# mila-iqia/diffusion_for_multi_scale_molecular_dynamics

Hardware: AMD Instinct MI355X
Metric: sampled structures/sec (1000-step predictor-corrector SDE sampling) (higher is better)
Workload: dtype f32 (per-edge matrix products as split-f16 hi/lo x3 MFMA terms with f32 accumulation: 22-bit products; state, updates, reductions and every other layer in f32)

## Files before the change

diffusion_for_multi_scale_molecular_dynamics_amd/csrc/mdx_egnn_chain.hip:

```cpp
#include <hip/hip_runtime.h>
#include <stdint.h>

#include <type_traits>

#include "../../include/mdx_hip.h"

namespace {

typedef _Float16 half8 __attribute__((ext_vector_type(8)));
typedef _Float16 half2v __attribute__((ext_vector_type(2)));
typedef float f32x16 __attribute__((ext_vector_type(16)));
typedef float f32x4 __attribute__((ext_vector_type(4)));
typedef __attribute__((address_space(3))) char lds_c;
typedef __attribute__((address_space(3))) float lds_f;
typedef __attribute__((address_space(1))) const char gbl_c;

constexpr int kWave = 64;
constexpr int kWaves = 4;
constexpr int kTileEdges = 32 * kWaves;
constexpr int kFastD = 6;
constexpr int kRing = 4;
constexpr int kScaleSlots = MDX_EGNN_CHAIN_MAX_LAYERS + 4;
constexpr int kMaxPositions = MDX_EGNN_CHAIN_MAX_LAYERS + 2;
constexpr int kEnds = kScaleSlots - 1;
// ... 995 lines not shown
            }
        };
        auto finish_rows = [&](Act<H, PREC>& y, Act<H, PREC>& u) {
            epilogue_elements<H, PREC>(NT - 1, 0, 16, pend, y, sc_prev, true, amax);
            flush_max(layers);
            const bool project = MODE == 3 && p.proj_out != nullptr;
            const float kOut = end_factor(2);
            int64_t row[NS];
            if constexpr (MODE == 3) {
#pragma unroll
                for (int es = 0; es < NS; ++es) row[es] = p.residual ? source_row(es, false) : e[es];
            }
#pragma unroll
            for (int q8 = 0; q8 < H / 8; ++q8) {
                const int t = q8 >> 2, q = q8 & 3, es = L::es(q), off = 32 * t + L::fb(q, h);
                f32x4 v = get4<H>(y, t, q);
#pragma unroll
                for (int i = 0; i < 4; ++i) v[i] *= kOut;
                if constexpr (SPLIT) {
#pragma unroll
                    for (int i = 0; i < 4; ++i) out_of_range = out_of_range || (is_live(es) && !(__builtin_fabsf(v[i]) <= 3.0e38f));
                }
                if (is_live(es)) {
                    if (p.residual) {
                        const f32x4 r4 = *(const f32x4*)(p.residual + (MODE == 3 ? row[es] : e[es]) * p.ld_in + off);
#pragma unroll
                        for (int i = 0; i < 4; ++i) v[i] = r4[i] + v[i];
                    }
                    *(f32x4*)(p.rows_out + e[es] * H + off) = v;
                }
                if ((q8 & 7) == 7) __builtin_amdgcn_sched_barrier(0);
            }
            ch.stores_count = stores_issued(H / 8);
            if constexpr (MODE == 3) {
                if (project) {
                    asm volatile("s_waitcnt vmcnt(0)" ::: "memory");
                    const float kIn = end_factor(3);
#pragma unroll
                    for (int q8 = 0; q8 < H / 8; ++q8) {
                        const int es = L::es(q8 & 3), off = 32 * (q8 >> 2) + L::fb(q8 & 3, h);
                        const f32x4 a = *(const f32x4*)(p.rows_out + e[es] * H + off);
                        note4(a[0] * kIn, a[1] * kIn, a[2] * kIn, a[3] * kIn);
                        put_pair<H>(u, q8 >> 2, 4 * (q8 & 3), a[0] * kIn, a[1] * kIn);
                        put_pair<H>(u, q8 >> 2, 4 * (q8 & 3) + 2, a[2] * kIn, a[3] * kIn);
                        if ((q8 & 15) == 15) __builtin_amdgcn_sched_barrier(0);
                    }
                    flush_max(layers + 1);
#pragma unroll 1
                    for (int t2 = 0; t2 < 2 * NT; ++t2) {
                        if constexpr (C::SPREAD) ch.scalar_addresses();
                        const f32x16 acc = run_tile(u, false, 0, u, t2 + 1 < 2 * NT ? nullptr : par, sc_prev);
                        const float to_out = load_scale(layers + t2 / NT).out;
#pragma unroll
                        for (int q = 0; q < 4; ++q) {
                            const int es = L::es(q);
                            const f32x4 v = {acc[4 * q] * to_out, acc[4 * q + 1] * to_out, acc[4 * q + 2] * to_out, acc[4 * q + 3] * to_out};
                            if constexpr (SPLIT) {
#pragma unroll
                                for (int i = 0; i < 4; ++i) out_of_range = out_of_range || (is_live(es) && !(__builtin_fabsf(v[i]) <= 3.0e38f));
                            }
                            if (is_live(es)) *(f32x4*)(p.proj_out + e[es] * 2 * H + 32 * t2 + L::fb(q, h)) = v;
                        }
                        ch.stores_count = stores_issued(4);
                    }
                }
            }
        };
        int l_first = 1;
        if constexpr (MODE == 3) {
#pragma unroll
            for (int t = 0; t < NT; ++t) {
                const f32x16 acc = run_tile(xa, false, 0, xa, t + 1 < NT ? par + 32 * (t + 1) : nullptr, sc_prev);
                park(xb, t, acc);
            }
            const float kIn = end_factor(1);
#pragma unroll
            for (int q8 = 0; q8 < H / 8; ++q8) {
                const int es = L::es(q8 & 3), off = 32 * (q8 >> 2) + L::fb(q8 & 3, h);
                const f32x4 a = *(const f32x4*)(p.rows_in2 + e[es] * p.ld_in2 + off);
                if constexpr (SPLIT) {
                    put_pair<H>(xa, q8 >> 2, 4 * (q8 & 3), a[0] * kIn, a[1] * kIn);
                    put_pair<H>(xa, q8 >> 2, 4 * (q8 & 3) + 2, a[2] * kIn, a[3] * kIn);
                } else {
                    note4(a[0] * kIn, a[1] * kIn, a[2] * kIn, a[3] * kIn);
#pragma unroll
                    for (int i = 0; i < 4; ++i) put<H>(xa, q8 >> 2, 4 * (q8 & 3) + i, a[i] * kIn);
                }
                if ((q8 & 15) == 15) __builtin_amdgcn_sched_barrier(0);
            }
            flush_max(0);
            acc_next = unpark(xb, 0);
#pragma unroll
            for (int t = 0; t < NT; ++t) {
                const lds_f* after = t + 1 < NT ? nullptr : par + 2 * H;
                pend = run_tile(xa, t > 0, t - 1, xb, after, sc_prev);
                if (t + 1 < NT) acc_next = unpark(xb, t + 1);
            }
            l_first = 2;
        } else {
            layer(std::true_type{}, xa, xb, 0);
        }
        bool done = false;
        if constexpr (MODE == 1) {
            if (layers == 1) {
                finish_rows(xb, xa);
                done = true;
            }
        }
        if (!done) {
            auto step_layer = [&](Act<H, PREC>& in, Act<H, PREC>& out, int l) {
                if constexpr (ATT) {
                    if (l == p.n_message) {
                        gate_messages(in, l);
                        reload_prefetch(par + l * H);
                        layer(std::true_type{}, in, out, l);
                    } else {
                        layer(std::false_type{}, in, out, l);
                    }
                } else {
                    layer(std::false_type{}, in, out, l);
                }
            };
            for (int l = l_first;;) {
                step_layer(xb, xa, l);
                if (!ROWS && l == p.n_message) {
                    if constexpr (MODE == 2) {
                        MDX_STAMP_ALWAYS(30);
                        ch.stores_count = aggregate_pieces(xb);
                        reload_prefetch(l + 1 < layers ? par + (l + 1) * H : nullptr);
                        MDX_STAMP_ALWAYS(31);
                    } else {
                        store_messages(xb);
                    }
                }
                if (++l >= layers) {
                    if constexpr (!ROWS) head_tile(xa);
                    else finish_rows(xa, xb);
                    break;
                }
                step_layer(xa, xb, l);
                if (!ROWS && l == p.n_message) {
                    if constexpr (MODE == 2) {
                        MDX_STAMP_ALWAYS(30);
                        ch.stores_count = aggregate_pieces(xa);
                        reload_prefetch(l + 1 < layers ? par + (l + 1) * H : nullptr);
                        MDX_STAMP_ALWAYS(31);
                    } else {
                        store_messages(xa);
                    }
                }
                if (++l >= layers) {
                    if constexpr (!ROWS) head_tile(xb);
                    else finish_rows(xb, xa);
                    break;
                }
            }
        }
    }
    asm volatile("s_waitcnt vmcnt(0)" ::: "memory");
    MDX_STAMP_ALWAYS(22);
    MDX_STAMP_REALTIME(23);
    if constexpr (SPLIT) {
        if (p.status && out_of_range) atomicOr(p.status, MDX_STATUS_EGNN_F16_RANGE);
    } else {
        __syncthreads();
        if (p.act_max && (int)threadIdx.x < layers + 2 && max_table[threadIdx.x]) atomicMax(p.act_max + threadIdx.x, max_table[threadIdx.x]);
    }
}

struct PackArgs {
    const float* w[MDX_EGNN_CHAIN_MAX_LAYERS];
    const float* w_out;
    int layers, H, precision;
    uint32_t tied;
    int32_t* exps;
    void* image;
};

__global__ __launch_bounds__(256) void egnn_chain_maxabs_kernel(PackArgs p)
{
    const int l = blockIdx.y;
    const bool head = l == p.layers;
    const float* w = head ? p.w_out : p.w[l];
    const int64_t n = head ? p.H : (int64_t)p.H * p.H;
    uint32_t m = 0;
    if (w)
        for (int64_t i = blockIdx.x * (int64_t)blockDim.x + threadIdx.x; i < n; i += (int64_t)gridDim.x * blockDim.x) {
            const uint32_t b = __builtin_bit_cast(uint32_t, w[i]) & 0x7fffffffu;
            if (b < 0x7f800000u && b > m) m = b;
        }
    for (int d = 32; d >= 1; d >>= 1) {
        const uint32_t o = (uint32_t)__shfl_xor((int)m, d);
        m = o > m ? o : m;
    }
    if ((threadIdx.x & 63) == 0 && m) atomicMax((uint32_t*)p.exps + l, m);
}
__global__ void egnn_chain_exponents_kernel(PackArgs p)
{
    if (blockIdx.x || threadIdx.x) return;
    for (int l = 0; l <= p.layers; ++l) {
        const uint32_t b = ((const uint32_t*)p.exps)[l];
        int a = 0;
        if (b) {
            const int e = (int)(b >> 23) - 127;
            a = 13 - (e < -126 ? -126 : e);
            a = a > 40 ? 40 : (a < -40 ? -40 : a);
        }
        p.exps[l] = a;
    }
    for (int l = 1; l < p.layers; ++l)
        if (p.tied >> l & 1u) {
            int lo = l - 1;
            while (lo > 0 && (p.tied >> lo & 1u)) --lo;
            int a = p.exps[lo];
            for (int k = lo + 1; k <= l; ++k) a = p.exps[k] < a ? p.exps[k] : a;
            for (int k = lo; k <= l; ++k) p.exps[k] = a;
        }
}

constexpr int kMinActExp = -14;
__global__ void egnn_chain_act_exponents_kernel(uint32_t* maxima, int count, int32_t* exps)
{
    if (blockIdx.x || threadIdx.x) return;
    for (int q = 0; q < count; ++q) {
        const uint32_t b = maxima[q] & 0x7fffffffu;
        maxima[q] = 0;
        if (!b) continue;
        const int e = b >= 0x7f800000u ? 127 : (int)(b >> 23) - 127;
        int c = 12 - e;
        c = c > kActExp<1> ? kActExp<1> : (c < kMinActExp ? kMinActExp : c);
        if (c < exps[q]) exps[q] = c;
    }
}

__global__ __launch_bounds__(256) void egnn_chain_pack_kernel(PackArgs p)
{
    const int H = p.H, NT = H / 32;
    const int64_t per_layer = (int64_t)H * H;
    const int64_t total = per_layer * p.layers + 32 * H;
    for (int64_t idx = blockIdx.x * (int64_t)blockDim.x + threadIdx.x; idx < total; idx += (int64_t)gridDim.x * blockDim.x) {
        const int l = (int)(idx / per_layer);
        int64_t r = idx - l * per_layer;
        const int t = (int)(r / (32 * H));
        r -= (int64_t)t * 32 * H;
        (void)NT;
        const bool head = l == p.layers;
        auto weight = [&](int n, int k) -> float {
            if (head) return (n == 0 && p.w_out) ? p.w_out[k] : 0.0f;
            return p.w[l][(int64_t)n * H + k];
        };
        if (p.precision == 0) {
            const int q = (int)(r / 256), lane = (int)(r % 256) / 4, i = (int)(r % 4);
            const int n = 32 * t + (lane & 31), k = 8 * q + 4 * (lane >> 5) + i;
            ((float*)p.image)[idx] = weight(n, k);
        } else {
            const int s = (int)(r / 512), lane = (int)(r % 512) / 8, j = (int)(r % 8);
            const int n = p.precision == 1 ? 32 * t + (lane & 31) : 32 * t + 16 * (s & 1) + (lane & 15);
            const int k = p.precision == 1 ? 16 * s + 8 * (j >> 2) + 4 * (lane >> 5) + (j & 3)
                                           : 32 * (s >> 1) + 16 * (j >> 2) + 4 * (lane >> 4) + (j & 3);
            const float v = weight(n, k) * pow2_bits(p.exps[l]);
            const _Float16 hi = (_Float16)v;
            const _Float16 lo = (_Float16)(v - (float)hi);
            _Float16* chunk = (_Float16*)((char*)p.image + ((int64_t)l * (H / 32) + t) * ((int64_t)H * 32 * 4));
            chunk[s * 1024 + lane * 8 + j] = hi;
            chunk[s * 1024 + 512 + lane * 8 + j] = lo;
        }
    }
}

__device__ __forceinline__ float coord_head_value(float s, int flags) { return (flags & MDX_EGNN_COORD_TANH) ? tanhf(s) : s; }
__device__ __forceinline__ float normalize_factor(float r2) { return tanhf(r2) / sqrtf(r2 + 1.0e-16f); }

__global__ __launch_bounds__(256) void egnn_coord_aggregate_kernel(const float* __restrict__ s, const float* __restrict__ coord,
                                                                   const int64_t* __restrict__ edges,
                                                                   const int64_t* __restrict__ offsets,
                                                                   const int64_t* __restrict__ degree, int64_t n_nodes, int D,
                                                                   int mean, int flags, float* __restrict__ out)
{
    const int64_t total = n_nodes * D;
    for (int64_t idx = blockIdx.x * (int64_t)blockDim.x + threadIdx.x; idx < total; idx += (int64_t)gridDim.x * blockDim.x) {
        const int64_t node = idx / D;
        const int k = (int)(idx - node * D);
        const int64_t e0 = offsets[node], deg = degree[node];
        const float ci = coord[idx];
        float acc = 0.0f;
        for (int64_t e = e0; e < e0 + deg; ++e) {
            const int64_t dst = edges[2 * e + 1];
            float diff = ci - coord[dst * D + k];
            if (flags & MDX_EGNN_COORD_NORMALIZE) {
                float r2 = 0.0f;
                for (int j = 0; j < D; ++j) {
                    const float dj = coord[node * D + j] - coord[dst * D + j];
                    r2 += dj * dj;
                }
                diff = normalize_factor(r2) * diff;
            }
            acc += diff * coord_head_value(s[e], flags);
        }
        if (mean && deg > 0) acc = acc / (float)deg;
        out[idx] = ci + acc;
    }
}

__global__ __launch_bounds__(256) void segment_combine_kernel(const float* __restrict__ pieces, const int64_t* __restrict__ offsets,
                                                              const int64_t* __restrict__ degree, int64_t n_nodes, int H,
                                                              int mean, float* __restrict__ out, const float* __restrict__ left,
                                                              int64_t boundary_rows)
{
    const int lane = threadIdx.x % kWave;
    const int64_t wave = (blockIdx.x * (int64_t)blockDim.x + threadIdx.x) / kWave;
    const int64_t n_waves = ((int64_t)gridDim.x * blockDim.x) / kWave;
    const int quads = H >> 2;
    for (int64_t node = wave; node < n_nodes; node += n_waves) {
        const int64_t e0 = offsets[node], deg = degree[node], e1 = e0 + deg;
        const float count = (mean && deg > 0) ? (float)deg : 1.0f;
        const int64_t last_row = ((e1 - 1) & 15) == 15 ? ((e1 - 1) >> 4) : boundary_rows + node;
        for (int q = lane; q < quads; q += kWave) {
            f32x4 acc = {0.0f, 0.0f, 0.0f, 0.0f};
            for (int64_t e = e0 | 15; e < e1 - 1; e += 16) acc += reinterpret_cast<const f32x4*>(pieces + (e >> 4) * H)[q];
            if (deg > 0) acc += reinterpret_cast<const f32x4*>(pieces + last_row * H)[q];
            if (mean) acc = acc / count;
            if (left) {
                reinterpret_cast<f32x4*>(out + node * 2 * H)[q] = reinterpret_cast<const f32x4*>(left + node * H)[q];
                reinterpret_cast<f32x4*>(out + node * 2 * H + H)[q] = acc;
            } else {
                reinterpret_cast<f32x4*>(out + node * H)[q] = acc;
            }
        }
    }
}

__global__ __launch_bounds__(256) void egnn_node_gather_kernel(const float* __restrict__ pieces, const int64_t* __restrict__ offsets,
                                                               const int64_t* __restrict__ degree, int64_t n_nodes, int H,
                                                               int mean_messages, float* __restrict__ out,
                                                               const float* __restrict__ left, int64_t boundary_rows,
                                                               const float* __restrict__ s, const float* __restrict__ coord,
                                                               const int64_t* __restrict__ edges, int D, int mean_coords,
                                                               int flags, float* __restrict__ coord_out)
{
    const int lane = threadIdx.x % kWave;
    const int64_t wave = (blockIdx.x * (int64_t)blockDim.x + threadIdx.x) / kWave;
    const int64_t n_waves = ((int64_t)gridDim.x * blockDim.x) / kWave;
    const int quads = H >> 2;
    for (int64_t node = wave; node < n_nodes; node += n_waves) {
        const int64_t e0 = offsets[node], deg = degree[node], e1 = e0 + deg;
        float part[8] = {0, 0, 0, 0, 0, 0, 0, 0}, ci[8];
#pragma unroll
        for (int k = 0; k < 8; ++k) ci[k] = k < D ? coord[node * D + k] : 0.0f;
        for (int64_t e = e0 + lane; e < e1; e += kWave) {
            const int64_t dst = edges[2 * e + 1];
            const float se = coord_head_value(s[e], flags);
            if (flags & MDX_EGNN_COORD_NORMALIZE) {
                float diff[8], r2 = 0.0f;
#pragma unroll
                for (int k = 0; k < 8; ++k) {
                    diff[k] = k < D ? ci[k] - coord[dst * D + k] : 0.0f;
                    if (k < D) r2 += diff[k] * diff[k];
                }
                const float f = normalize_factor(r2);
#pragma unroll
                for (int k = 0; k < 8; ++k)
                    if (k < D) part[k] += (f * diff[k]) * se;
            } else {
#pragma unroll
                for (int k = 0; k < 8; ++k)
                    if (k < D) part[k] += (ci[k] - coord[dst * D + k]) * se;
            }
        }
        const float count = (mean_messages && deg > 0) ? (float)deg : 1.0f;
        const int64_t last_row = ((e1 - 1) & 15) == 15 ? ((e1 - 1) >> 4) : boundary_rows + node;
        for (int q = lane; pieces && q < quads; q += kWave) {
            f32x4 acc = {0.0f, 0.0f, 0.0f, 0.0f};
            for (int64_t e = e0 | 15; e < e1 - 1; e += 16) acc += reinterpret_cast<const f32x4*>(pieces + (e >> 4) * H)[q];
            if (deg > 0) acc += reinterpret_cast<const f32x4*>(pieces + last_row * H)[q];
            if (mean_messages) acc = acc / count;
            if (left) {
                reinterpret_cast<f32x4*>(out + node * 2 * H)[q] = reinterpret_cast<const f32x4*>(left + node * H)[q];
                reinterpret_cast<f32x4*>(out + node * 2 * H + H)[q] = acc;
            } else {
                reinterpret_cast<f32x4*>(out + node * H)[q] = acc;
            }
        }
#pragma unroll
        for (int k = 0; k < 8; ++k) {
            if (k < D) {
                float v = part[k];
                v += __builtin_bit_cast(float, __builtin_amdgcn_update_dpp(0, __builtin_bit_cast(int, v), 0x111, 0xf, 0xf, false));
                v += __builtin_bit_cast(float, __builtin_amdgcn_update_dpp(0, __builtin_bit_cast(int, v), 0x112, 0xf, 0xf, false));
                v += __builtin_bit_cast(float, __builtin_amdgcn_update_dpp(0, __builtin_bit_cast(int, v), 0x114, 0xf, 0xf, false));
                v += __builtin_bit_cast(float, __builtin_amdgcn_update_dpp(0, __builtin_bit_cast(int, v), 0x118, 0xf, 0xf, false));
                v += __builtin_bit_cast(float, __builtin_amdgcn_update_dpp(0, __builtin_bit_cast(int, v), 0x142, 0xa, 0xf, false));
                v += __builtin_bit_cast(float, __builtin_amdgcn_update_dpp(0, __builtin_bit_cast(int, v), 0x143, 0xc, 0xf, false));
                part[k] = __builtin_bit_cast(float, __builtin_amdgcn_readlane(__builtin_bit_cast(int, v), 63));
            }
        }
        if (lane < D) {
            float total = 0.0f, mine = 0.0f;
#pragma unroll
            for (int k = 0; k < 8; ++k) {
                if (k == lane) { total = part[k]; mine = ci[k]; }
            }
            if (mean_coords && deg > 0) total = total / (float)deg;
            coord_out[node * D + lane] = mine + total;
        }
    }
}

template <int H, int PREC, int MODE, bool ATT = false>
int launch_chain(const ChainArgs& a, int layers, hipStream_t st)
{
    using C = Chain<H, PREC>;
    size_t lds = (size_t)kRing * C::CHUNK + sizeof(float) * ((size_t)layers * H + 2 * H + 4 * kScaleSlots) +
                 sizeof(int) * kWaves * 32 + sizeof(uint32_t) * kMaxPositions;
    if (ATT) lds = ((lds + 15) & ~(size_t)15) + sizeof(float) * (H + 4);
    static bool granted[64] = {};
    int dev = 0;
    if (hipGetDevice(&dev) != hipSuccess || dev < 0 || dev >= 64) return MDX_ERR_HIP;
    if (lds > 64 * 1024 && !granted[dev]) {
        if (hipFuncSetAttribute((const void*)egnn_edge_chain_kernel<H, PREC, MODE, ATT>, hipFuncAttributeMaxDynamicSharedMemorySize,
                                160 * 1024) != hipSuccess)
            return MDX_ERR_HIP;
        granted[dev] = true;
    }
    if (lds > 160 * 1024) return MDX_ERR_UNSUPPORTED;
    int64_t tiles = (a.n_edges + kTileEdges - 1) / kTileEdges;
    int cus = 256;
    if (hipDeviceGetAttribute(&cus, hipDeviceAttributeMultiprocessorCount, dev) != hipSuccess) cus = 256;
    const unsigned grid = (unsigned)(tiles < cus ? tiles : cus);
    hipLaunchKernelGGL((egnn_edge_chain_kernel<H, PREC, MODE, ATT>), dim3(grid), dim3(kWaves * kWave), lds, st, a);
    return hipGetLastError() == hipSuccess ? MDX_OK : MDX_ERR_HIP;
}

}

extern "C" int mdx_chain_launch_attention(const void* args, int hidden, int precision, int layers, mdx_stream_t stream);

#ifdef MDX_CHAIN_ATTENTION_UNIT
extern "C" int mdx_chain_launch_attention(const void* args, int hidden, int precision, int layers, mdx_stream_t stream)
{
    const ChainArgs& a = *static_cast<const ChainArgs*>(args);
    hipStream_t st = reinterpret_cast<hipStream_t>(stream);
#define MDX_ATT_CASE(HH) \
    case HH: return precision == 0 ? launch_chain<HH, 0, 2, true>(a, layers, st) : (precision == 1 ? launch_chain<HH, 1, 2, true>(a, layers, st) : launch_chain<HH, 2, 2, true>(a, layers, st));
    switch (hidden) {
        MDX_ATT_CASE(32)
        MDX_ATT_CASE(64)
        MDX_ATT_CASE(128)
        MDX_ATT_CASE(256)
    }
#undef MDX_ATT_CASE
    return MDX_ERR_UNSUPPORTED;
}
#endif

#ifndef MDX_CHAIN_NO_ENTRY_POINTS
extern "C" {

int64_t mdx_egnn_chain_image_bytes(int hidden, int n_layers)
{
    if (hidden < 32 || (hidden % 32) || n_layers < 1) return -1;
    return ((int64_t)n_layers * hidden * hidden + 32 * hidden) * 4;
}

int mdx_egnn_chain_pack(const float* const* weights_host, int n_layers, const float* w_out, int hidden, int precision,
                        uint32_t tied_layers, void* image_out, int32_t* exponents_out, mdx_stream_t stream)
{
    if (!weights_host || !image_out || n_layers < 1 || precision < 0 || precision > 2) return MDX_ERR_INVALID_ARG;
    if (precision >= 1 && !exponents_out) return MDX_ERR_INVALID_ARG;
    if (n_layers > MDX_EGNN_CHAIN_MAX_LAYERS) return MDX_ERR_UNSUPPORTED;
    if (hidden != 32 && hidden != 64 && hidden != 128 && hidden != 256) return MDX_ERR_UNSUPPORTED;
    PackArgs a{};
    for (int l = 0; l < n_layers; ++l) {
        if (!weights_host[l]) return MDX_ERR_INVALID_ARG;
        a.w[l] = weights_host[l];
    }
    a.w_out = w_out;
    a.layers = n_layers; a.H = hidden; a.precision = precision; a.image = image_out;
    a.tied = tied_layers; a.exps = exponents_out;
    hipStream_t st = reinterpret_cast<hipStream_t>(stream);
    if (exponents_out) {
        if (hipMemsetAsync(exponents_out, 0, sizeof(int32_t) * (n_layers + 1), st) != hipSuccess) return MDX_ERR_HIP;
        if (precision >= 1) {
            hipLaunchKernelGGL(egnn_chain_maxabs_kernel, dim3(32, (unsigned)n_layers + 1), dim3(256), 0, st, a);
            hipLaunchKernelGGL(egnn_chain_exponents_kernel, dim3(1), dim3(64), 0, st, a);
        }
    }
    const int64_t total = (int64_t)n_layers * hidden * hidden + 32 * hidden;
    int64_t blocks = (total + 255) / 256;
    if (blocks > 4096) blocks = 4096;
    hipLaunchKernelGGL(egnn_chain_pack_kernel, dim3((unsigned)blocks), dim3(256), 0, st, a);
    return hipGetLastError() == hipSuccess ? MDX_OK : MDX_ERR_HIP;
}

int mdx_egnn_edge_chain(const mdx_egnn_chain_t* c, const float* node_proj, const float* coord, int coord_dimension,
                        const int64_t* edges, int64_t n_edges, const int64_t* n_edges_dev, float* messages_out,
                        float* edge_scalar_out, uint32_t* status, mdx_stream_t stream)
{
    return mdx_egnn_edge_chain_keyed(c, node_proj, coord, coord_dimension, edges, n_edges, n_edges_dev, messages_out,
                                     edge_scalar_out, status, nullptr, nullptr, stream);
}

int mdx_egnn_edge_chain_keyed(const mdx_egnn_chain_t* c, const float* node_proj, const float* coord, int coord_dimension,
                              const int64_t* edges, int64_t n_edges, const int64_t* n_edges_dev, float* messages_out,
                              float* edge_scalar_out, uint32_t* status, const uint32_t* table_key, const float* sigma,
                              mdx_stream_t stream)
{
    if (!c || n_edges < 0 || coord_dimension < 1) return MDX_ERR_INVALID_ARG;
    if (table_key && (!sigma || c->message_mode != MDX_EGNN_MESSAGES_ROWS || c->attention_weight)) return MDX_ERR_INVALID_ARG;
    if (c->n_message_layers < 1 || c->n_coord_layers < 1 || (c->precision < 0 || c->precision > 2) ||
        (c->message_mode != MDX_EGNN_MESSAGES_ROWS && c->message_mode != MDX_EGNN_MESSAGES_PIECE_SUMS))
        return MDX_ERR_INVALID_ARG;
    if (c->n_message_layers + c->n_coord_layers > MDX_EGNN_CHAIN_MAX_LAYERS) return MDX_ERR_UNSUPPORTED;
    if (c->hidden != 32 && c->hidden != 64 && c->hidden != 128 && c->hidden != 256) return MDX_ERR_UNSUPPORTED;
    if (n_edges == 0) return MDX_OK;
    if (!c->weight_image || !c->biases || !c->bias_in || !c->w_radial || !node_proj || !coord || !edges ||
        !messages_out || !edge_scalar_out || (c->precision >= 1 && !c->weight_exponents))
        return MDX_ERR_INVALID_ARG;
    ChainArgs a{};
    a.image = (const char*)c->weight_image; a.biases = c->biases; a.bias_in = c->bias_in; a.w_radial = c->w_radial;
    a.exps = c->weight_exponents;
    a.act_exps = c->activation_exponents; a.act_max = c->activation_maxima;
    a.node_proj = node_proj; a.coord = coord; a.edges = edges; a.n_edges_dev = n_edges_dev;
    a.n_edges = n_edges; a.n_message = c->n_message_layers; a.n_coord = c->n_coord_layers; a.D = coord_dimension;
    a.messages = messages_out; a.edge_scalar = edge_scalar_out; a.status = status;
    a.piece_sums = c->message_mode == MDX_EGNN_MESSAGES_PIECE_SUMS;
    if ((c->attention_weight == nullptr) != (c->attention_bias == nullptr)) return MDX_ERR_INVALID_ARG;
    a.att_w = c->attention_weight; a.att_b = c->attention_bias;
    a.table_key = table_key; a.table_sigma = table_key ? sigma : nullptr;
#ifdef MDX_CHAIN_STAMPS
    if (status && hipMemsetAsync((char*)status + 4095 * 8, 0, 8, reinterpret_cast<hipStream_t>(stream)) != hipSuccess) return MDX_ERR_HIP;
    a.stamp_buf = status;
    a.status = nullptr;
#endif
    const int layers = a.n_message + a.n_coord;
    hipStream_t st = reinterpret_cast<hipStream_t>(stream);
    if (a.att_w) return a.piece_sums ? mdx_chain_launch_attention(&a, c->hidden, c->precision, layers, stream) : MDX_ERR_UNSUPPORTED;
#define MDX_CHAIN_MODE(HH, MM, AA) (c->precision == 0 ? launch_chain<HH, 0, MM, AA>(a, layers, st) : (c->precision == 1 ? launch_chain<HH, 1, MM, AA>(a, layers, st) : launch_chain<HH, 2, MM, AA>(a, layers, st)))
#define MDX_CHAIN_CASE(HH)                                                                                            \
    case HH:                                                                                                          \
        return a.piece_sums ? MDX_CHAIN_MODE(HH, 2, false) : MDX_CHAIN_MODE(HH, 0, false);
    switch (c->hidden) {
        MDX_CHAIN_CASE(32)
        MDX_CHAIN_CASE(64)
        MDX_CHAIN_CASE(128)
        MDX_CHAIN_CASE(256)
    }
#undef MDX_CHAIN_CASE
#undef MDX_CHAIN_MODE
    return MDX_ERR_UNSUPPORTED;
}

int mdx_egnn_chain_adapt_activation_exponents(uint32_t* maxima_inout, int count, int32_t* exponents_inout, mdx_stream_t stream)
{
    if (!maxima_inout || !exponents_inout || count < 1 || count > MDX_EGNN_CHAIN_MAX_LAYERS + 2) return MDX_ERR_INVALID_ARG;
    hipLaunchKernelGGL(egnn_chain_act_exponents_kernel, dim3(1), dim3(64), 0, reinterpret_cast<hipStream_t>(stream), maxima_inout,
                       count, exponents_inout);
    return hipGetLastError() == hipSuccess ? MDX_OK : MDX_ERR_HIP;
}

int64_t mdx_egnn_piece_rows(int64_t n_edges, int64_t n_nodes)
{
    if (n_edges < 0 || n_nodes < 0) return -1;
    return ((n_edges + 15) >> 4) + n_nodes;
}

int mdx_segment_combine(const float* pieces, int64_t n_edges, const int64_t* offsets, const int64_t* degree, int64_t n_nodes,
                        int H, int mean, const float* left, float* out, mdx_stream_t stream)
{
    if (n_nodes < 0 || H < 4 || n_edges < 0) return MDX_ERR_INVALID_ARG;
    if (H & 3) return MDX_ERR_UNSUPPORTED;
    if (n_nodes == 0) return MDX_OK;
    if (!pieces || !offsets || !degree || !out) return MDX_ERR_INVALID_ARG;
    int64_t blocks = (n_nodes * kWave + 255) / 256;
    if (blocks > 16384) blocks = 16384;
    hipLaunchKernelGGL(segment_combine_kernel, dim3((unsigned)blocks), dim3(256), 0, reinterpret_cast<hipStream_t>(stream),
                       pieces, offsets, degree, n_nodes, H, mean, out, left, (n_edges + 15) >> 4);
    return hipGetLastError() == hipSuccess ? MDX_OK : MDX_ERR_HIP;
}

int mdx_egnn_node_gather(const float* pieces, int64_t n_edges, const int64_t* offsets, const int64_t* degree, int64_t n_nodes,
                         int H, int mean_messages, const float* left, float* out, const float* edge_scalar, const float* coord,
                         int coord_dimension, const int64_t* edges, int mean_coords, int coord_flags, float* coord_out,
                         mdx_stream_t stream)
{
    if (n_nodes < 0 || H < 4 || n_edges < 0 || coord_dimension < 1) return MDX_ERR_INVALID_ARG;
    if (coord_flags & ~(MDX_EGNN_COORD_NORMALIZE | MDX_EGNN_COORD_TANH)) return MDX_ERR_INVALID_ARG;
    if ((H & 3) || coord_dimension > 8) return MDX_ERR_UNSUPPORTED;
    if (n_nodes == 0) return MDX_OK;
    if (!offsets || !degree || !edge_scalar || !coord || !edges || !coord_out) return MDX_ERR_INVALID_ARG;
    if (pieces ? !out : (out || left)) return MDX_ERR_INVALID_ARG;
    int64_t blocks = (n_nodes * kWave + 255) / 256;
    if (blocks > 16384) blocks = 16384;
    hipLaunchKernelGGL(egnn_node_gather_kernel, dim3((unsigned)blocks), dim3(256), 0, reinterpret_cast<hipStream_t>(stream),
                       pieces, offsets, degree, n_nodes, H, mean_messages, out, left, (n_edges + 15) >> 4, edge_scalar, coord, edges,
                       coord_dimension, mean_coords, coord_flags, coord_out);
    return hipGetLastError() == hipSuccess ? MDX_OK : MDX_ERR_HIP;
}

int mdx_mlp_chain_rows(const mdx_egnn_chain_t* c, const float* x, const float* residual, int64_t n_rows,
                       const int64_t* n_rows_dev, float* out, uint32_t* status, mdx_stream_t stream)
{
    if (!c || n_rows < 0) return MDX_ERR_INVALID_ARG;
    if (c->n_message_layers < 1 || c->n_coord_layers != 0 || (c->precision < 0 || c->precision > 2)) return MDX_ERR_INVALID_ARG;
    if (c->n_message_layers > MDX_EGNN_CHAIN_MAX_LAYERS) return MDX_ERR_UNSUPPORTED;
    if (c->hidden != 32 && c->hidden != 64 && c->hidden != 128 && c->hidden != 256) return MDX_ERR_UNSUPPORTED;
    if (n_rows == 0) return MDX_OK;
    if (!c->weight_image || !c->biases || !x || !out || (c->precision >= 1 && !c->weight_exponents)) return MDX_ERR_INVALID_ARG;
    ChainArgs a{};
    a.image = (const char*)c->weight_image; a.biases = c->biases; a.exps = c->weight_exponents;
    a.act_exps = c->activation_exponents; a.act_max = c->activation_maxima;
    a.n_edges_dev = n_rows_dev; a.n_edges = n_rows; a.n_message = c->n_message_layers; a.n_coord = 0; a.D = 0;
    a.rows_in = x; a.residual = residual; a.rows_out = out; a.status = status; a.ld_in = c->hidden;
    const int layers = a.n_message;
    hipStream_t st = reinterpret_cast<hipStream_t>(stream);
#define MDX_ROWS_CASE(HH)                                                                          \
    case HH: return c->precision == 0 ? launch_chain<HH, 0, 1>(a, layers, st) : (c->precision == 1 ? launch_chain<HH, 1, 1>(a, layers, st) : launch_chain<HH, 2, 1>(a, layers, st));
    switch (c->hidden) {
        MDX_ROWS_CASE(32)
        MDX_ROWS_CASE(64)
        MDX_ROWS_CASE(128)
        MDX_ROWS_CASE(256)
    }
#undef MDX_ROWS_CASE
    return MDX_ERR_UNSUPPORTED;
}

static int node_mlp_rows(const mdx_egnn_chain_t* c, const float* node_in, int64_t ld, const float* agg, int64_t ld_agg,
                         int add_residual, int64_t n_rows, const int64_t* n_rows_dev, float* out, float* proj_out,
                         uint32_t* status, mdx_stream_t stream, const int64_t* row_class = nullptr, int n_classes = 0);

int mdx_node_mlp_rows(const mdx_egnn_chain_t* c, const float* node_in, int add_residual, int64_t n_rows,
                      const int64_t* n_rows_dev, float* out, float* proj_out, uint32_t* status, mdx_stream_t stream)
{
    if (!c) return MDX_ERR_INVALID_ARG;
    return node_mlp_rows(c, node_in, 2 * (int64_t)c->hidden, node_in ? node_in + c->hidden : nullptr, 2 * (int64_t)c->hidden,
                         add_residual, n_rows, n_rows_dev, out, proj_out, status, stream);
}

int mdx_node_mlp_rows_split(const mdx_egnn_chain_t* c, const float* h, const float* agg, int add_residual, int64_t n_rows,
                            const int64_t* n_rows_dev, float* out, float* proj_out, uint32_t* status, mdx_stream_t stream)
{
    if (!c) return MDX_ERR_INVALID_ARG;
    return node_mlp_rows(c, h, c->hidden, agg, c->hidden, add_residual, n_rows, n_rows_dev, out, proj_out, status, stream);
}

int mdx_node_mlp_rows_indexed(const mdx_egnn_chain_t* c, const float* class_rows, int n_classes, const int64_t* row_class,
                              const float* agg, int add_residual, int64_t n_rows, const int64_t* n_rows_dev, float* out,
                              float* proj_out, uint32_t* status, mdx_stream_t stream)
{
    if (!c || n_classes < 1 || (n_rows > 0 && !row_class)) return MDX_ERR_INVALID_ARG;
    return node_mlp_rows(c, class_rows, c->hidden, agg, c->hidden, add_residual, n_rows, n_rows_dev, out, proj_out, status, stream,
                         row_class, n_classes);
}

static int node_mlp_rows(const mdx_egnn_chain_t* c, const float* node_in, int64_t ld, const float* agg, int64_t ld_agg,
                         int add_residual, int64_t n_rows, const int64_t* n_rows_dev, float* out, float* proj_out,
                         uint32_t* status, mdx_stream_t stream, const int64_t* row_class, int n_classes)
{
    if (!c || n_rows < 0) return MDX_ERR_INVALID_ARG;
    if (c->n_message_layers < 3 || c->n_coord_layers != 0 || (c->precision < 0 || c->precision > 2)) return MDX_ERR_INVALID_ARG;
    if (c->n_message_layers > MDX_EGNN_CHAIN_MAX_LAYERS) return MDX_ERR_UNSUPPORTED;
    if (c->hidden != 32 && c->hidden != 64 && c->hidden != 128 && c->hidden != 256) return MDX_ERR_UNSUPPORTED;
    if (n_rows == 0) return MDX_OK;
    if (!c->weight_image || !c->biases || !node_in || !agg || !out || (c->precision >= 1 && !c->weight_exponents)) return MDX_ERR_INVALID_ARG;
    ChainArgs a{};
    a.image = (const char*)c->weight_image; a.biases = c->biases; a.exps = c->weight_exponents;
    a.act_exps = c->activation_exponents; a.act_max = c->activation_maxima;
    a.n_edges_dev = n_rows_dev; a.n_edges = n_rows; a.n_message = c->n_message_layers; a.n_coord = 0; a.D = 0;
    a.rows_in = node_in; a.residual = add_residual ? node_in : nullptr; a.rows_out = out; a.status = status;
    a.ld_in = ld; a.rows_in2 = agg; a.ld_in2 = ld_agg;
    a.proj_out = proj_out;
    a.row_class = row_class; a.n_classes = n_classes;
    if (proj_out && c->n_message_layers + 2 > MDX_EGNN_CHAIN_MAX_LAYERS) return MDX_ERR_UNSUPPORTED;
    const int layers = a.n_message;
    hipStream_t st = reinterpret_cast<hipStream_t>(stream);
#define MDX_NODE_CASE(HH)                                                                          \
    case HH: return c->precision == 0 ? launch_chain<HH, 0, 3>(a, layers, st) : (c->precision == 1 ? launch_chain<HH, 1, 3>(a, layers, st) : launch_chain<HH, 2, 3>(a, layers, st));
    switch (c->hidden) {
        MDX_NODE_CASE(32)
        MDX_NODE_CASE(64)
        MDX_NODE_CASE(128)
        MDX_NODE_CASE(256)
    }
#undef MDX_NODE_CASE
    return MDX_ERR_UNSUPPORTED;
}

int mdx_egnn_coord_aggregate(const float* edge_scalar, const float* coord, int coord_dimension, const int64_t* edges,
                             const int64_t* offsets, const int64_t* degree, int64_t n_nodes, int mean, int coord_flags,
                             float* coord_out, mdx_stream_t stream)
{
    if (n_nodes < 0 || coord_dimension < 1) return MDX_ERR_INVALID_ARG;
    if (coord_flags & ~(MDX_EGNN_COORD_NORMALIZE | MDX_EGNN_COORD_TANH)) return MDX_ERR_INVALID_ARG;
    if (n_nodes == 0) return MDX_OK;
    if (!edge_scalar || !coord || !edges || !offsets || !degree || !coord_out) return MDX_ERR_INVALID_ARG;
    int64_t blocks = (n_nodes * coord_dimension + 255) / 256;
    if (blocks > 16384) blocks = 16384;
    hipLaunchKernelGGL(egnn_coord_aggregate_kernel, dim3((unsigned)blocks), dim3(256), 0, reinterpret_cast<hipStream_t>(stream),
                       edge_scalar, coord, edges, offsets, degree, n_nodes, coord_dimension, mean, coord_flags, coord_out);
    return hipGetLastError() == hipSuccess ? MDX_OK : MDX_ERR_HIP;
}

}
#endif
```

Baseline: 21.76.

## Restructure EGNN node gather to issue all per-node loads up front

Rewrites the node gather kernel so each wave first issues every load for a node: offsets, edge destinations, edge scalars, the partial-sum rows and the neighbour coordinates. The sums are done afterwards, which removes the serial load-then-add loops. Nodes with degree up to 64 and a small number of piece rows take this path; others fall back to the old per-node routine. It also adds a D=6 specialization that uses 8-byte vector coordinate loads, a node-group template (default one node per wave), and a lower block cap. Register use rises and the code gets more complex, with a fallback path for large-degree nodes.

```diff
diff --git a/diffusion_for_multi_scale_molecular_dynamics_amd/csrc/mdx_egnn_chain.hip b/diffusion_for_multi_scale_molecular_dynamics_amd/csrc/mdx_egnn_chain.hip
--- a/diffusion_for_multi_scale_molecular_dynamics_amd/csrc/mdx_egnn_chain.hip
+++ b/diffusion_for_multi_scale_molecular_dynamics_amd/csrc/mdx_egnn_chain.hip
@@ -1321,6 +1321,28 @@
     }
 }
 
+__device__ __forceinline__ void combine_node_pieces(const float* __restrict__ pieces, int64_t boundary_rows, int64_t node,
+                                                    int64_t e0, int64_t deg, int H, int mean, float* __restrict__ out,
+                                                    const float* __restrict__ left, int q_first)
+{
+    const int quads = H >> 2;
+    const int64_t e1 = e0 + deg;
+    const float count = (mean && deg > 0) ? (float)deg : 1.0f;
+    const int64_t last_row = ((e1 - 1) & 15) == 15 ? ((e1 - 1) >> 4) : boundary_rows + node;
+    for (int q = q_first; q < quads; q += kWave) {
+        f32x4 acc = {0.0f, 0.0f, 0.0f, 0.0f};
+        for (int64_t e = e0 | 15; e < e1 - 1; e += 16) acc += reinterpret_cast<const f32x4*>(pieces + (e >> 4) * H)[q];
+        if (deg > 0) acc += reinterpret_cast<const f32x4*>(pieces + last_row * H)[q];
+        if (mean) acc = acc / count;
+        if (left) {
+            reinterpret_cast<f32x4*>(out + node * 2 * H)[q] = reinterpret_cast<const f32x4*>(left + node * H)[q];
+            reinterpret_cast<f32x4*>(out + node * 2 * H + H)[q] = acc;
+        } else {
+            reinterpret_cast<f32x4*>(out + node * H)[q] = acc;
+        }
+    }
+}
+
 __global__ __launch_bounds__(256) void segment_combine_kernel(const float* __restrict__ pieces, const int64_t* __restrict__ offsets,
                                                               const int64_t* __restrict__ degree, int64_t n_nodes, int H,
                                                               int mean, float* __restrict__ out, const float* __restrict__ left,
@@ -1329,98 +1351,249 @@
     const int lane = threadIdx.x % kWave;
     const int64_t wave = (blockIdx.x * (int64_t)blockDim.x + threadIdx.x) / kWave;
     const int64_t n_waves = ((int64_t)gridDim.x * blockDim.x) / kWave;
+    for (int64_t node = wave; node < n_nodes; node += n_waves)
+        combine_node_pieces(pieces, boundary_rows, node, offsets[node], degree[node], H, mean, out, left, lane);
+}
+
+template <int CTRL, int ROWS>
+__device__ __forceinline__ float gather_dpp_step(float v)
+{
+    return v + __builtin_bit_cast(float, __builtin_amdgcn_update_dpp(0, __builtin_bit_cast(int, v), CTRL, ROWS, 0xf, false));
+}
+template <int N>
+__device__ __forceinline__ void gather_wave_totals(float (&v)[N], int D)
+{
+#define MDX_GATHER_STEP(CTRL, ROWS)                                                  \
+    _Pragma("unroll") for (int i = 0; i < N; ++i)                                    \
+        if ((i & 7) < D) v[i] = gather_dpp_step<CTRL, ROWS>(v[i]);
+    MDX_GATHER_STEP(0x111, 0xf)
+    MDX_GATHER_STEP(0x112, 0xf)
+    MDX_GATHER_STEP(0x114, 0xf)
+    MDX_GATHER_STEP(0x118, 0xf)
+    MDX_GATHER_STEP(0x142, 0xa)
+    MDX_GATHER_STEP(0x143, 0xc)
+#undef MDX_GATHER_STEP
+#pragma unroll
+    for (int i = 0; i < N; ++i)
+        if ((i & 7) < D) v[i] = __builtin_bit_cast(float, __builtin_amdgcn_readlane(__builtin_bit_cast(int, v[i]), 63));
+}
+
+__device__ __forceinline__ void gather_one_node(int64_t node, int lane, const float* __restrict__ pieces,
+                                                const int64_t* __restrict__ offsets, const int64_t* __restrict__ degree, int H,
+                                                int mean_messages, float* __restrict__ out, const float* __restrict__ left,
+                                                int64_t boundary_rows, const float* __restrict__ s,
+                                                const float* __restrict__ coord, const int64_t* __restrict__ edges, int D,
+                                                int mean_coords, int flags, float* __restrict__ coord_out)
+{
+    const int64_t e0 = offsets[node], deg = degree[node], e1 = e0 + deg;
+    float part[8] = {0, 0, 0, 0, 0, 0, 0, 0}, ci[8];
+#pragma unroll
+    for (int k = 0; k < 8; ++k) ci[k] = k < D ? coord[node * D + k] : 0.0f;
+    for (int64_t e = e0 + lane; e < e1; e += kWave) {
+        const int64_t dst = edges[2 * e + 1];
+        const float se = coord_head_value(s[e], flags);
+        if (flags & MDX_EGNN_COORD_NORMALIZE) {
+            float diff[8], r2 = 0.0f;
+#pragma unroll
+            for (int k = 0; k < 8; ++k) {
+                diff[k] = k < D ? ci[k] - coord[dst * D + k] : 0.0f;
+                if (k < D) r2 += diff[k] * diff[k];
+            }
+            const float f = normalize_factor(r2);
+#pragma unroll
+            for (int k = 0; k < 8; ++k)
+                if (k < D) part[k] += (f * diff[k]) * se;
+        } else {
+#pragma unroll
+            for (int k = 0; k < 8; ++k)
+                if (k < D) part[k] += (ci[k] - coord[dst * D + k]) * se;
+        }
+    }
+    if (pieces) combine_node_pieces(pieces, boundary_rows, node, e0, deg, H, mean_messages, out, left, lane);
+    gather_wave_totals(part, D);
+    if (lane < D) {
+        float total = 0.0f, mine = 0.0f;
+#pragma unroll
+        for (int k = 0; k < 8; ++k) {
+            if (k == lane) { total = part[k]; mine = ci[k]; }
+        }
+        if (mean_coords && deg > 0) total = total / (float)deg;
+        coord_out[node * D + lane] = mine + total;
+    }
+}
+
+#ifdef MDX_GATHER_NODES
+constexpr int kGatherNodes = MDX_GATHER_NODES, kGatherPieces = MDX_GATHER_PIECES, kGatherWaves = MDX_GATHER_WAVES;
+#else
+constexpr int kGatherNodes = 1;
+constexpr int kGatherPieces = 4;
+constexpr int kGatherWaves = 1;
+#endif
+constexpr int kGatherMaxBlocks = 4096;
+constexpr int kGatherThreads = 256;
+
+template <int DC>
+__global__ __launch_bounds__(kGatherThreads, kGatherWaves) void egnn_node_gather_kernel(
+    const float* __restrict__ pieces, const int64_t* __restrict__ offsets, const int64_t* __restrict__ degree, int64_t n_nodes, int H,
+    int mean_messages, float* __restrict__ out, const float* __restrict__ left, int64_t boundary_rows, const float* __restrict__ s,
+    const float* __restrict__ coord, const int64_t* __restrict__ edges, int D_runtime, int mean_coords, int flags,
+    float* __restrict__ coord_out)
+{
+    constexpr int G = kGatherNodes, P = kGatherPieces;
+    typedef float f32x2 __attribute__((ext_vector_type(2)));
+    const int D = DC ? DC : D_runtime;
+    const int lane = threadIdx.x % kWave;
+    const int64_t wave = blockIdx.x * (int64_t)(blockDim.x / kWave) + __builtin_amdgcn_readfirstlane((int)(threadIdx.x / kWave));
+    const int64_t n_waves = (int64_t)gridDim.x * (blockDim.x / kWave);
     const int quads = H >> 2;
-    for (int64_t node = wave; node < n_nodes; node += n_waves) {
-        const int64_t e0 = offsets[node], deg = degree[node], e1 = e0 + deg;
-        const float count = (mean && deg > 0) ? (float)deg : 1.0f;
-        const int64_t last_row = ((e1 - 1) & 15) == 15 ? ((e1 - 1) >> 4) : boundary_rows + node;
-        for (int q = lane; q < quads; q += kWave) {
-            f32x4 acc = {0.0f, 0.0f, 0.0f, 0.0f};
-            for (int64_t e = e0 | 15; e < e1 - 1; e += 16) acc += reinterpret_cast<const f32x4*>(pieces + (e >> 4) * H)[q];
-            if (deg > 0) acc += reinterpret_cast<const f32x4*>(pieces + last_row * H)[q];
-            if (mean) acc = acc / count;
+    for (int64_t node0 = wave * G; node0 < n_nodes; node0 += n_waves * G) {
+        if (node0 + G > n_nodes) {
+#pragma nounroll
+            for (int64_t node = node0; node < n_nodes; ++node)
+                gather_one_node(node, lane, pieces, offsets, degree, H, mean_messages, out, left, boundary_rows, s, coord, edges, D,
+                                mean_coords, flags, coord_out);
+            break;
+        }
+        int64_t e0[G], d64[G];
+#pragma unroll
+        for (int m = 0; m < G; ++m) {
+            e0[m] = offsets[node0 + m];
+            d64[m] = degree[node0 + m];
+        }
+        int64_t first_row[G], last_row[G];
+        int deg[G], n_boundary[G], n_rows[G];
+        unsigned other_way = 0;
+#pragma unroll
+        for (int m = 0; m < G; ++m) {
+            const int64_t e1 = e0[m] + d64[m], b0 = e0[m] | 15;
+            const int64_t boundary = b0 < e1 - 1 ? ((e1 - 2 - b0) >> 4) + 1 : 0;
+            const bool fits = d64[m] <= kWave && !(pieces && boundary + 1 > P);
+            if (!fits) other_way |= 1u << m;
+            deg[m] = fits ? (int)d64[m] : 0;
+            n_boundary[m] = fits ? (int)boundary : 0;
+            n_rows[m] = fits ? (int)boundary + (d64[m] > 0 ? 1 : 0) : 0;
+            first_row[m] = b0 >> 4;
+            last_row[m] = ((e1 - 1) & 15) == 15 ? ((e1 - 1) >> 4) : boundary_rows + node0 + m;
+        }
+        int64_t dst[G];
+        float se[G];
+#pragma unroll
+        for (int m = 0; m < G; ++m) {
+            if (lane < deg[m]) {
+                const int64_t e = e0[m] + lane;
+                dst[m] = edges[2 * e + 1];
+                se[m] = s[e];
+            }
+        }
+        f32x4 row[G][P];
+        const int column = lane < quads ? lane : quads - 1;
+        if (pieces) {
+#pragma unroll
+            for (int m = 0; m < G; ++m) {
+#pragma unroll
+                for (int p = 0; p < P; ++p)
+                    if (p < n_rows[m])
+                        row[m][p] = reinterpret_cast<const f32x4*>(pieces + (p < n_boundary[m] ? first_row[m] + p : last_row[m]) * H)[column];
+            }
+        }
+        float cj[G][8];
+#pragma unroll
+        for (int m = 0; m < G; ++m) {
+            if (lane < deg[m]) {
+                if (DC == 6) {
+                    const f32x2* r = reinterpret_cast<const f32x2*>(coord + dst[m] * 6);
+                    const f32x2 a = r[0], b = r[1], c = r[2];
+                    cj[m][0] = a.x; cj[m][1] = a.y; cj[m][2] = b.x; cj[m][3] = b.y; cj[m][4] = c.x; cj[m][5] = c.y;
+                } else {
+#pragma unroll
+                    for (int k = 0; k < 8; ++k)
+                        if (k < D) cj[m][k] = coord[dst[m] * D + k];
+                }
+            }
+        }
+        float ci[G][8];
+#pragma unroll
+        for (int m = 0; m < G; ++m)
+#pragma unroll
+            for (int k = 0; k < 8; ++k) ci[m][k] = k < D ? coord[(node0 + m) * D + k] : 0.0f;
+        if (pieces) {
+            f32x4 acc[G];
+#pragma unroll
+            for (int m = 0; m < G; ++m) {
+                acc[m] = f32x4{0.0f, 0.0f, 0.0f, 0.0f};
+#pragma unroll
+                for (int p = 0; p < P; ++p)
+                    if (p < n_rows[m]) acc[m] += row[m][p];
+                const float count = (mean_messages && deg[m] > 0) ? (float)deg[m] : 1.0f;
+                if (mean_messages) acc[m] = acc[m] / count;
+            }
+            const int64_t ld = left ? 2 * (int64_t)H : H;
+#pragma unroll
+            for (int m = 0; m < G; ++m)
+                if (!(other_way >> m & 1) && lane < quads) reinterpret_cast<f32x4*>(out + (node0 + m) * ld + (ld - H))[lane] = acc[m];
             if (left) {
-                reinterpret_cast<f32x4*>(out + node * 2 * H)[q] = reinterpret_cast<const f32x4*>(left + node * H)[q];
-                reinterpret_cast<f32x4*>(out + node * 2 * H + H)[q] = acc;
-            } else {
-                reinterpret_cast<f32x4*>(out + node * H)[q] = acc;
-            }
-        }
-    }
-}
-
-__global__ __launch_bounds__(256) void egnn_node_gather_kernel(const float* __restrict__ pieces, const int64_t* __restrict__ offsets,
-                                                               const int64_t* __restrict__ degree, int64_t n_nodes, int H,
-                                                               int mean_messages, float* __restrict__ out,
-                                                               const float* __restrict__ left, int64_t boundary_rows,
-                                                               const float* __restrict__ s, const float* __restrict__ coord,
-                                                               const int64_t* __restrict__ edges, int D, int mean_coords,
-                                                               int flags, float* __restrict__ coord_out)
-{
-    const int lane = threadIdx.x % kWave;
-    const int64_t wave = (blockIdx.x * (int64_t)blockDim.x + threadIdx.x) / kWave;
-    const int64_t n_waves = ((int64_t)gridDim.x * blockDim.x) / kWave;
-    const int quads = H >> 2;
-    for (int64_t node = wave; node < n_nodes; node += n_waves) {
-        const int64_t e0 = offsets[node], deg = degree[node], e1 = e0 + deg;
-        float part[8] = {0, 0, 0, 0, 0, 0, 0, 0}, ci[8];
-#pragma unroll
-        for (int k = 0; k < 8; ++k) ci[k] = k < D ? coord[node * D + k] : 0.0f;
-        for (int64_t e = e0 + lane; e < e1; e += kWave) {
-            const int64_t dst = edges[2 * e + 1];
-            const float se = coord_head_value(s[e], flags);
-            if (flags & MDX_EGNN_COORD_NORMALIZE) {
-                float diff[8], r2 = 0.0f;
+                f32x4 left_row[G];
+#pragma unroll
+                for (int m = 0; m < G; ++m)
+                    if (!(other_way >> m & 1)) left_row[m] = reinterpret_cast<const f32x4*>(left + (node0 + m) * H)[column];
+#pragma unroll
+                for (int m = 0; m < G; ++m)
+                    if (!(other_way >> m & 1) && lane < quads) reinterpret_cast<f32x4*>(out + (node0 + m) * ld)[lane] = left_row[m];
+            }
+            if (quads > kWave) {
+#pragma nounroll
+                for (int m = 0; m < G; ++m)
+                    if (!(other_way >> m & 1))
+                        combine_node_pieces(pieces, boundary_rows, node0 + m, offsets[node0 + m], degree[node0 + m], H, mean_messages,
+                                            out, left, kWave + lane);
+            }
+        }
+        float part[8 * G];
+#pragma unroll
+        for (int m = 0; m < G; ++m) {
+#pragma unroll
+            for (int k = 0; k < 8; ++k) part[8 * m + k] = 0.0f;
+            if (lane < deg[m]) {
+                const float sv = coord_head_value(se[m], flags);
+                if (flags & MDX_EGNN_COORD_NORMALIZE) {
+                    float diff[8], r2 = 0.0f;
+#pragma unroll
+                    for (int k = 0; k < 8; ++k) {
+                        diff[k] = k < D ? ci[m][k] - cj[m][k] : 0.0f;
+                        if (k < D) r2 += diff[k] * diff[k];
+                    }
+                    const float f = normalize_factor(r2);
+#pragma unroll
+                    for (int k = 0; k < 8; ++k)
+                        if (k < D) part[8 * m + k] += (f * diff[k]) * sv;
+                } else {
+#pragma unroll
+                    for (int k = 0; k < 8; ++k)
+                        if (k < D) part[8 * m + k] += (ci[m][k] - cj[m][k]) * sv;
+                }
+            }
+        }
+        gather_wave_totals(part, D);
+#pragma unroll
+        for (int m = 0; m < G; ++m) {
+            const int64_t node = node0 + m;
+            if (other_way >> m & 1) continue;
+            if (lane < D) {
+                float total = 0.0f, mine = 0.0f;
 #pragma unroll
                 for (int k = 0; k < 8; ++k) {
-                    diff[k] = k < D ? ci[k] - coord[dst * D + k] : 0.0f;
-                    if (k < D) r2 += diff[k] * diff[k];
-                }
-                const float f = normalize_factor(r2);
-#pragma unroll
-                for (int k = 0; k < 8; ++k)
-                    if (k < D) part[k] += (f * diff[k]) * se;
-            } else {
-#pragma unroll
-                for (int k = 0; k < 8; ++k)
-                    if (k < D) part[k] += (ci[k] - coord[dst * D + k]) * se;
-            }
-        }
-        const float count = (mean_messages && deg > 0) ? (float)deg : 1.0f;
-        const int64_t last_row = ((e1 - 1) & 15) == 15 ? ((e1 - 1) >> 4) : boundary_rows + node;
-        for (int q = lane; pieces && q < quads; q += kWave) {
-            f32x4 acc = {0.0f, 0.0f, 0.0f, 0.0f};
-            for (int64_t e = e0 | 15; e < e1 - 1; e += 16) acc += reinterpret_cast<const f32x4*>(pieces + (e >> 4) * H)[q];
-            if (deg > 0) acc += reinterpret_cast<const f32x4*>(pieces + last_row * H)[q];
-            if (mean_messages) acc = acc / count;
-            if (left) {
-                reinterpret_cast<f32x4*>(out + node * 2 * H)[q] = reinterpret_cast<const f32x4*>(left + node * H)[q];
-                reinterpret_cast<f32x4*>(out + node * 2 * H + H)[q] = acc;
-            } else {
-                reinterpret_cast<f32x4*>(out + node * H)[q] = acc;
-            }
-        }
-#pragma unroll
-        for (int k = 0; k < 8; ++k) {
-            if (k < D) {
-                float v = part[k];
-                v += __builtin_bit_cast(float, __builtin_amdgcn_update_dpp(0, __builtin_bit_cast(int, v), 0x111, 0xf, 0xf, false));
-                v += __builtin_bit_cast(float, __builtin_amdgcn_update_dpp(0, __builtin_bit_cast(int, v), 0x112, 0xf, 0xf, false));
-                v += __builtin_bit_cast(float, __builtin_amdgcn_update_dpp(0, __builtin_bit_cast(int, v), 0x114, 0xf, 0xf, false));
-                v += __builtin_bit_cast(float, __builtin_amdgcn_update_dpp(0, __builtin_bit_cast(int, v), 0x118, 0xf, 0xf, false));
-                v += __builtin_bit_cast(float, __builtin_amdgcn_update_dpp(0, __builtin_bit_cast(int, v), 0x142, 0xa, 0xf, false));
-                v += __builtin_bit_cast(float, __builtin_amdgcn_update_dpp(0, __builtin_bit_cast(int, v), 0x143, 0xc, 0xf, false));
-                part[k] = __builtin_bit_cast(float, __builtin_amdgcn_readlane(__builtin_bit_cast(int, v), 63));
-            }
-        }
-        if (lane < D) {
-            float total = 0.0f, mine = 0.0f;
-#pragma unroll
-            for (int k = 0; k < 8; ++k) {
-                if (k == lane) { total = part[k]; mine = ci[k]; }
-            }
-            if (mean_coords && deg > 0) total = total / (float)deg;
-            coord_out[node * D + lane] = mine + total;
+                    if (k == lane) { total = part[8 * m + k]; mine = ci[m][k]; }
+                }
+                if (mean_coords && deg[m] > 0) total = total / (float)deg[m];
+                coord_out[node * D + lane] = mine + total;
+            }
+        }
+        if (other_way) {
+#pragma nounroll
+            for (int m = 0; m < G; ++m)
+                if (other_way >> m & 1)
+                    gather_one_node(node0 + m, lane, pieces, offsets, degree, H, mean_messages, out, left, boundary_rows, s, coord,
+                                    edges, D, mean_coords, flags, coord_out);
         }
     }
 }
@@ -1608,11 +1781,13 @@
     if (n_nodes == 0) return MDX_OK;
     if (!offsets || !degree || !edge_scalar || !coord || !edges || !coord_out) return MDX_ERR_INVALID_ARG;
     if (pieces ? !out : (out || left)) return MDX_ERR_INVALID_ARG;
-    int64_t blocks = (n_nodes * kWave + 255) / 256;
-    if (blocks > 16384) blocks = 16384;
-    hipLaunchKernelGGL(egnn_node_gather_kernel, dim3((unsigned)blocks), dim3(256), 0, reinterpret_cast<hipStream_t>(stream),
-                       pieces, offsets, degree, n_nodes, H, mean_messages, out, left, (n_edges + 15) >> 4, edge_scalar, coord, edges,
-                       coord_dimension, mean_coords, coord_flags, coord_out);
+    const int64_t groups = (n_nodes + kGatherNodes - 1) / kGatherNodes;
+    int64_t blocks = (groups * kWave + kGatherThreads - 1) / kGatherThreads;
+    if (blocks > kGatherMaxBlocks) blocks = kGatherMaxBlocks;
+    const bool fast_rows = coord_dimension == 6 && (reinterpret_cast<uintptr_t>(coord) & 7) == 0;
+    hipLaunchKernelGGL(fast_rows ? egnn_node_gather_kernel<6> : egnn_node_gather_kernel<0>, dim3((unsigned)blocks), dim3(kGatherThreads), 0,
+                       reinterpret_cast<hipStream_t>(stream), pieces, offsets, degree, n_nodes, H, mean_messages, out, left,
+                       (n_edges + 15) >> 4, edge_scalar, coord, edges, coord_dimension, mean_coords, coord_flags, coord_out);
     return hipGetLastError() == hipSuccess ? MDX_OK : MDX_ERR_HIP;
 }
 
```

Result: no change. 21.81, median of 6 (+0.2%).
